# 86885974647565434342125458569795756674/torch.distributed.pipeline.sync.Pipe

Hardware: AMD Instinct MI355X
Metric: tokens/sec for 12-layer Transformer at PP=N (pipeline-parallel training) (higher is better)
Workload: dtype bf16

## Files before the change

mipipe/csrc/bindings.cpp:

```cpp
#include <torch/extension.h>
#include <ATen/hip/HIPContext.h>
#include <ATen/hip/HIPGeneratorImpl.h>
#include <ATen/core/Generator.h>
#include <ATen/hip/impl/HIPGuardImplMasqueradingAsCUDA.h>
#include <ATen/hip/impl/HIPStreamMasqueradingAsCUDA.h>

#include <mutex>
#include <optional>
#include <tuple>

#include "kernels/kernels.h"
#include "runtime/ipc.h"
#include "runtime/runtime.h"

namespace py = pybind11;
using at::Tensor;

namespace mipipe {
namespace {

#define MP_CHECK(cond, ...) TORCH_CHECK(cond, "mipipe: ", __VA_ARGS__)

hipStream_t cur_stream(const Tensor& t) { return at::hip::getCurrentHIPStreamMasqueradingAsCUDA(t.device().index()).stream(); }

// ... 1642 lines not shown
  MP_CHECK(t.scalar_type() == at::kFloat, who, ": sinks must be fp32, got ", t.scalar_type());
  MP_CHECK(t.dim() == 1 && t.size(0) == a.H, who, ": sinks must be [H] = [", a.H, "], one per query head");
  MP_CHECK(t.device() == q.device(), who, ": sinks must be on q's device");
  MP_CHECK(t.is_contiguous(), who, ": sinks must be contiguous");
  a.sinks = static_cast<const float*>(t.data_ptr());
}

void fill_options(AttnArgs& a, const char* who, const Tensor& q, bool causal, int64_t kv_len, int64_t window,
                  double softcap, const std::optional<Tensor>& doc_bounds, const std::optional<Tensor>& sinks) {
  attn_docs(a, who, doc_bounds, causal, q);
  attn_sinks(a, who, sinks, q);
  a.window = attn_window(who, window, causal, q, a.S);
  a.softcap = attn_softcap(who, softcap, q);
  MP_CHECK(kv_len == 0 || (q.scalar_type() == at::kFloat && kv_len > 0 && kv_len <= a.S), who,
           ": kv_len (a key-length bound) is for fp32, 0 < kv_len <= S");
  a.kv_len = (int)kv_len;
}

std::tuple<Tensor, Tensor, int64_t, int64_t, Tensor> py_attention_fwd(Tensor q, Tensor k, Tensor v, bool causal,
                                                                      double p, double scale, int64_t kv_len,
                                                                      std::optional<Tensor> words, int64_t words_seed,
                                                                      int64_t words_offset, int64_t window, double softcap,
                                                                      std::optional<Tensor> doc_bounds,
                                                                      std::optional<Tensor> sinks) {
  AttnArgs a;
  fill_qkv(a, q, k, v);
  fill_options(a, "attention", q, causal, kv_len, window, softcap, doc_bounds, sinks);
  MP_CHECK(p >= 0.0 && p < 1.0, "attention: bad dropout p");
  at::hip::HIPGuardMasqueradingAsCUDA guard(q.device());
  auto o = at::empty({a.B, a.S, a.H, a.D}, q.options());
  auto lse = at::empty({a.B, a.H, a.S}, q.options().dtype(at::kFloat));
  uint64_t seed = 0, offset = 0;
  if (p > 0.0) std::tie(seed, offset) = philox_draw(q.device(), 4);
  a.o = o.data_ptr(); a.sb_o = o.stride(0); a.ld_o = o.stride(1); a.sh_o = o.stride(2);
  a.lse = ptr<float>(lse);
  a.scale = (float)scale; a.p = (float)p; a.seed = seed; a.offset = offset; a.causal = causal;
  Tensor bits = at::empty({0}, q.options().dtype(at::kInt));
  if (q.scalar_type() == at::kFloat) {
    attention_f32_fwd(a, cur_stream(q));
  } else if (runs_long(a, q)) {
    bool reuse = false;
    if (p > 0.0) {
      const std::vector<int64_t> shape = {(int64_t)a.B * a.H, a.S / 32, a.S};
      reuse = words && words->defined() && words->sizes() == at::IntArrayRef(shape) &&
              words->scalar_type() == at::kInt && words->is_contiguous() && words->device() == q.device() &&
              (uint64_t)words_seed == seed && (uint64_t)words_offset == offset;
      bits = reuse ? *words : at::empty(shape, q.options().dtype(at::kInt));
      a.dmask = reinterpret_cast<uint32_t*>(bits.data_ptr());
    }
    if (reuse) attention_long_fwd_words(a, cur_stream(q));
    else attention_long_fwd(a, cur_stream(q));
  } else {
    attention_fwd(a, cur_stream(q));
// ... 288 lines not shown
  m.def("moe_combine_bwd", &py_moe_combine_bwd, py::arg("dy"), py::arg("ye"), py::arg("gate"), py::arg("src"));
  m.def("bias_act_fwd", &py_bias_act_fwd);
  m.def("softcap_fwd", &py_softcap_fwd, py::arg("x"), py::arg("cap"), py::arg("out") = py::none());
  m.def("softcap_bwd", &py_softcap_bwd, py::arg("dy"), py::arg("y"), py::arg("cap"), py::arg("out") = py::none());
  m.def("bias_act_bwd", &py_bias_act_bwd, py::arg("dy"), py::arg("saved"), py::arg("bias"), py::arg("act"),
        py::arg("p"), py::arg("seed"), py::arg("offset"), py::arg("need_dbias"), py::arg("dbias_acc") = py::none());
  m.def("column_sum", &py_column_sum, py::arg("x"), py::arg("out") = py::none(), py::arg("accumulate") = false);
  m.def("cross_entropy_fwd", &py_ce_fwd, py::arg("logits"), py::arg("target"), py::arg("ignore_index"),
        py::arg("t_offset") = 0);
  m.def("cross_entropy_bwd", &py_ce_bwd, py::arg("logits"), py::arg("target"), py::arg("lse"), py::arg("scale"),
        py::arg("ignore_index"), py::arg("row_scale") = py::none(), py::arg("out") = py::none(),
        py::arg("zero_pad") = false, py::arg("t_offset") = 0, py::arg("stat_out") = py::none());
  m.def("cross_entropy_mean_fwd", &py_ce_mean_fwd, py::arg("logits"), py::arg("target"), py::arg("ignore_index"));
  m.def("vsplit_head_fwd", &py_vsplit_head_fwd);
  m.def("vsplit_tail_fwd", &py_vsplit_tail_fwd);
  m.def("embedding_fwd", &py_embed_fwd);
  m.def("embedding_bwd", &py_embed_bwd, py::arg("tokens"), py::arg("dout"), py::arg("dweight"), py::arg("scale"),
        py::arg("p"), py::arg("seed"), py::arg("offset"), py::arg("dpe") = py::none());
  m.def("attention_supported", [](int64_t S, int64_t D) { return attention_supported((int)S, (int)D); });
  m.def("attention_f32_supported", [](int64_t S, int64_t D) { return attention_f32_supported((int)S, (int)D); });
  m.def("attention_fwd", &py_attention_fwd, py::arg("q"), py::arg("k"), py::arg("v"), py::arg("causal"), py::arg("p"),
        py::arg("scale"), py::arg("kv_len") = 0, py::arg("words") = py::none(), py::arg("words_seed") = 0,
        py::arg("words_offset") = 0, py::arg("window") = 0, py::arg("softcap") = 0.0,
        py::arg("doc_bounds") = py::none(), py::arg("sinks") = py::none());
  m.def("attention_bwd", &py_attention_bwd, py::arg("dout"), py::arg("q"), py::arg("k"), py::arg("v"), py::arg("o"),
        py::arg("lse"), py::arg("causal"), py::arg("p"), py::arg("scale"), py::arg("seed"), py::arg("offset"),
        py::arg("dq"), py::arg("dk"), py::arg("dv"), py::arg("bits") = py::none(), py::arg("kv_len") = 0,
        py::arg("window") = 0, py::arg("softcap") = 0.0, py::arg("doc_bounds") = py::none(),
        py::arg("sinks") = py::none(), py::arg("dsinks") = py::none(), py::arg("dsinks_accumulate") = false);
  m.def("attention_dsink", &py_attention_dsink, py::arg("lse"), py::arg("delta"), py::arg("sinks"), py::arg("dsinks"),
        py::arg("accumulate") = false);
  m.def("attention_long_supported", [](int64_t S, int64_t D) { return attention_long_supported((int)S, (int)D); });
  m.def("attention_long_set_fused_rng", &attention_long_set_fused_rng,
        "long-sequence attention: make the dropout keep words inside the forward kernel (true, default) or in a "
        "kernel of their own before it (false)");
  m.def("gemm_supported", &py_gemm_supported);
  m.def("gemm_f32_supported", &py_gemm_f32_supported);
  m.def("attention_set_fused_bwd", &attention_set_fused_bwd);
  m.def("gemm_set_rounds", &gemm_set_rounds,
        "multi-round GEMM grids whose last round is at most half full: 0 one launch, 1 (default) one launch per round "
        "of tiles when K >= 4096, 2 one launch per round at any K");
  m.def("gemm_set_splitk", &gemm_set_splitk, "split-K factor of under-filled long-K GEMMs: 0 off, 1 auto (default), n >= 2 forced");
  m.def("gemm_set_width", &gemm_set_width, "256-row GEMM block width: 0 auto (grid-quantisation rule), 128, 256");
  m.def("linear_fwd", &py_linear_fwd, py::arg("x"), py::arg("w"), py::arg("bias"), py::arg("act"), py::arg("p"),
        py::arg("save_preact"), py::arg("res") = py::none(), py::arg("xt") = py::none(),
        py::arg("aux_grad") = false, py::arg("bits") = py::none());
  m.def("linear_bits_ok",
        [](int64_t M, int64_t N, int64_t K, int64_t act, double p) {
          GemmArgs g;
          g.M = (int)M; g.N = (int)N; g.K = (int)K; g.act = (int)act; g.p = (float)p;
          g.a_kc = true; g.b_kc = true; g.epi = kEpiStoreAct;
          return gemm_supported(M, N, K) && gemm_bits_ok(g);
        },
        py::arg("M"), py::arg("N"), py::arg("K"), py::arg("act"), py::arg("p"),
        "whether linear_fwd can also write the ReLU output's nonzero mask as bits (kActReluBits)");
  m.def("gemm_emit_ok", &gemm_emit_ok, py::arg("act"), py::arg("p"), py::arg("aux"),
        "whether linear_fwd can also write x^T for this activation / dropout / pre-activation output");
  m.def("linear_wgrad_xt_segments", &py_linear_wgrad_xt_segments, py::arg("dys"), py::arg("xts"),
        py::arg("main_grad"), py::arg("accumulate") = true, py::arg("bias_grad") = py::none());
  m.def("linear_dgrad", &py_linear_dgrad, py::arg("dy"), py::arg("w"), py::arg("res") = py::none(),
        py::arg("out") = py::none(), py::arg("act") = 0, py::arg("saved") = py::none(), py::arg("p") = 0.0,
// ... 12 lines not shown
```

mipipe/csrc/kernels/attention.hip:

```cpp
#include <type_traits>

#include "common.h"
#include "kernels.h"

namespace mipipe {

namespace {

typedef __attribute__((ext_vector_type(4))) short s16x4;
typedef __attribute__((ext_vector_type(8))) short s16x8;
typedef __attribute__((address_space(3))) s16x4 lds_s16x4;

constexpr int kRows = 64;
constexpr int kThreads = 256;
constexpr float kLog2e = 1.4426950408889634f;

template <int D>
struct Img {
  static constexpr int kRowBytes = 2 * D;
  static constexpr int kChunks = D / 8;
  static constexpr int kBytes = kRows * kRowBytes;
  __device__ static __forceinline__ int f(int r) {
    if constexpr (kChunks >= 16) return (((r ^ (r >> 2)) & 1) << 1) | ((r & 2) << 1) | (r & 8);
    else if constexpr (kChunks == 8) return ((((r >> 1) ^ (r >> 2)) & 1) << 1) | ((r >> 1) & 4);
// ... 963 lines not shown
      dk[t2] = __builtin_amdgcn_mfma_f32_16x16x32_bf16(f1, frag_cols<D>(qimg, 16 * t2, 1, lane), dk[t2], 0, 0, 0);
    }
  }
  const DkvDst dst = dkv_dst<0>(blockIdx.y);
  bf16_t* dK = dst.dk;
  bf16_t* dV = dst.dv;
#pragma unroll
  for (int t2 = 0; t2 < ND; ++t2)
#pragma unroll
    for (int r = 0; r < 4; ++r) {
      const int64_t o = (int64_t)(key0 + r) * dst.ld + 16 * t2 + (lane & 15);
      dK[o] = f2bf(dk[t2][r] * a.scale);
      dV[o] = f2bf(dv[t2][r]);
    }
}

namespace shortseq {

constexpr int S = 128;
constexpr int kThreads = 512;
constexpr int kChunk = 64;
constexpr int kChunkImg = S * kChunk * 2;
constexpr int kSqImg = S * S * 2;
constexpr int kStageBytes = 3 * kChunkImg;
constexpr int kPOff = 4 * kChunkImg;
constexpr int kDsOff = kPOff + kSqImg;
constexpr int kSmem = kDsOff + kSqImg;
constexpr int kFwdPOff = 2 * kChunkImg;
constexpr int kFwdSmem = kFwdPOff + kSqImg;

__device__ __forceinline__ int coff(int r, int c16) { return Img<64>::off(r, c16); }
__device__ __forceinline__ int soff(int r, int c16) { return Img<128>::off(r, c16); }

__device__ __forceinline__ void load_chunk(const bf16_t* __restrict__ base, int64_t ld, int d0, int tid, uint4& v0,
                                           uint4& v1) {
  const int r = tid >> 3, c = tid & 7;
  v0 = *reinterpret_cast<const uint4*>(base + (int64_t)r * ld + d0 + 8 * c);
  v1 = *reinterpret_cast<const uint4*>(base + (int64_t)(r + 64) * ld + d0 + 8 * c);
}
__device__ __forceinline__ void store_chunk(char* img, int tid, const uint4& v0, const uint4& v1) {
  const int r = tid >> 3, c = tid & 7;
  *reinterpret_cast<uint4*>(img + coff(r, c)) = v0;
  *reinterpret_cast<uint4*>(img + coff(r + 64, c)) = v1;
}

__device__ __forceinline__ bf16x8 crow(const char* img, int rb, int s, int lane) {
  return *reinterpret_cast<const bf16x8*>(img + coff(rb + (lane & 15), 4 * s + (lane >> 4)));
}
__device__ __forceinline__ bf16x8 ccol(const char* img, int db, int s, int lane) {
  const int g = lane >> 4, q = (lane & 15) >> 2, p = lane & 3;
  const int r0 = 32 * s + 8 * g + q;
  const int c8 = (db >> 2) + p;
  const int o0 = coff(r0, c8 >> 1) + 8 * (c8 & 1);
  const int o1 = coff(r0 + 4, c8 >> 1) + 8 * (c8 & 1);
  const s16x4 lo = __builtin_amdgcn_ds_read_tr16_b64_v4i16((lds_s16x4*)(img + o0));
  const s16x4 hi = __builtin_amdgcn_ds_read_tr16_b64_v4i16((lds_s16x4*)(img + o1));
  return __builtin_bit_cast(bf16x8, __builtin_shufflevector(lo, hi, 0, 1, 2, 3, 4, 5, 6, 7));
}
__device__ __forceinline__ bf16x8 srow(const char* img, int rb, int s, int lane) {
  return *reinterpret_cast<const bf16x8*>(img + soff(rb + (lane & 15), 4 * s + (lane >> 4)));
}
__device__ __forceinline__ bf16x8 scol(const char* img, int ib, int s, int lane) {
  const int g = lane >> 4, q = (lane & 15) >> 2, p = lane & 3;
  const int r0 = 32 * s + 8 * g + q;
  const int c8 = (ib >> 2) + p;
  const int o0 = soff(r0, c8 >> 1) + 8 * (c8 & 1);
  const int o1 = soff(r0 + 4, c8 >> 1) + 8 * (c8 & 1);
  const s16x4 lo = __builtin_amdgcn_ds_read_tr16_b64_v4i16((lds_s16x4*)(img + o0));
  const s16x4 hi = __builtin_amdgcn_ds_read_tr16_b64_v4i16((lds_s16x4*)(img + o1));
  return __builtin_bit_cast(bf16x8, __builtin_shufflevector(lo, hi, 0, 1, 2, 3, 4, 5, 6, 7));
}

template <int D, bool CAUSAL>
__global__ void __launch_bounds__(kThreads, 1) attn_bwd_s128_kernel(AttnArgs a) {
  extern __shared__ __attribute__((aligned(16))) char smem[];
  const int tid = threadIdx.x, lane = tid & 63, wave = __builtin_amdgcn_readfirstlane(tid >> 6);
  const int bh = blockIdx.x;
  const int b = bh / a.H, h = bh % a.H;
  const int64_t boff = (int64_t)b * a.sb_qkv + (int64_t)h * a.sh_qkv;
  const int64_t koff = (int64_t)b * a.sb_qkv + (int64_t)kv_head(a, h) * a.sh_qkv;
  const bf16_t* Q = reinterpret_cast<const bf16_t*>(a.q) + boff;
  const bf16_t* K = reinterpret_cast<const bf16_t*>(a.k) + koff;
  const bf16_t* V = reinterpret_cast<const bf16_t*>(a.v) + koff;
  const bf16_t* dO = reinterpret_cast<const bf16_t*>(a.dout) + (int64_t)b * a.sb_o + (int64_t)h * a.sh_o;
  constexpr int NC = D / kChunk;

  f32x4 sacc[8], pacc[8];
#pragma unroll
  for (int j = 0; j < 8; ++j) sacc[j] = pacc[j] = f32x4{0.f, 0.f, 0.f, 0.f};
  const int myrow = wave * 16 + (lane & 15);
  const bf16_t* qrow = Q + (int64_t)myrow * a.ld_qkv;
  const bf16_t* drow = dO + (int64_t)myrow * a.ld_o;

  uint4 k0, k1, v0, v1;
  load_chunk(K, a.ld_qkv, 0, tid, k0, k1);
  load_chunk(V, a.ld_qkv, 0, tid, v0, v1);
  store_chunk(smem, tid, k0, k1);
  store_chunk(smem + kChunkImg, tid, v0, v1);
  __syncthreads();
#pragma unroll 1
  for (int c = 0; c < NC; ++c) {
    const char* kimg = smem + (c & 1) * 2 * kChunkImg;
    const char* vimg = kimg + kChunkImg;
    if (c + 1 < NC) {
      load_chunk(K, a.ld_qkv, (c + 1) * kChunk, tid, k0, k1);
      load_chunk(V, a.ld_qkv, (c + 1) * kChunk, tid, v0, v1);
    }
    bf16x8 qf[2], df[2];
#pragma unroll
    for (int s2 = 0; s2 < 2; ++s2) {
      qf[s2] = frag_global(qrow + c * kChunk, s2, lane);
      df[s2] = frag_global(drow + c * kChunk, s2, lane);
    }
#pragma unroll
    for (int s2 = 0; s2 < 2; ++s2)
#pragma unroll
      for (int j = 0; j < 8; ++j) {
        sacc[j] = __builtin_amdgcn_mfma_f32_16x16x32_bf16(qf[s2], crow(kimg, 16 * j, s2, lane), sacc[j], 0, 0, 0);
        pacc[j] = __builtin_amdgcn_mfma_f32_16x16x32_bf16(df[s2], crow(vimg, 16 * j, s2, lane), pacc[j], 0, 0, 0);
      }
    if (c + 1 < NC) {
      char* nimg = smem + ((c + 1) & 1) * 2 * kChunkImg;
      store_chunk(nimg, tid, k0, k1);
      store_chunk(nimg + kChunkImg, tid, v0, v1);
    }
    __syncthreads();
  }

  const int qrow0 = wave * 16 + 4 * (lane >> 4);
  const float sl2 = a.scale * kLog2e;
  const float pscale = a.p > 0.f ? 1.f / (1.f - a.p) : 1.f;
  float lse2[4];
#pragma unroll
  for (int r = 0; r < 4; ++r) lse2[r] = a.lse[(int64_t)bh * S + qrow0 + r] * kLog2e;
  float dsum[4] = {0.f, 0.f, 0.f, 0.f};
#pragma unroll
  for (int j = 0; j < 8; ++j) {
    const int key = 16 * j + (lane & 15);
    uint32_t w[4] = {0xFFFFFFFFu, 0xFFFFFFFFu, 0xFFFFFFFFu, 0xFFFFFFFFu};
    if (a.p > 0.f) {
      const uint4 mw = attn_mask_words(a, bh, qrow0 >> 2, key);
      w[0] = mw.x; w[1] = mw.y; w[2] = mw.z; w[3] = mw.w;
    }
#pragma unroll
    for (int r = 0; r < 4; ++r) {
      float pr = __builtin_amdgcn_exp2f(sacc[j][r] * sl2 - lse2[r]);
      if (CAUSAL && key > qrow0 + r) pr = 0.f;
      float dp = pacc[j][r];
      float pd = pr;
      if (a.p > 0.f) {
        const bool keep = w[r] >= a.threshold;
        dp = keep ? dp * pscale : 0.f;
        pd = keep ? pr * pscale : 0.f;
      }
      sacc[j][r] = pr;
      pacc[j][r] = dp;
      dsum[r] += pr * dp;
      *reinterpret_cast<bf16_t*>(smem + kPOff + soff(qrow0 + r, key >> 3) + 2 * (key & 7)) = f2bf(pd);
    }
  }
  float delta[4];
#pragma unroll
  for (int r = 0; r < 4; ++r) delta[r] = row_reduce_sum16(dsum[r]);
#pragma unroll
  for (int j = 0; j < 8; ++j) {
    const int key = 16 * j + (lane & 15);
#pragma unroll
    for (int r = 0; r < 4; ++r) {
      const float ds = sacc[j][r] * (pacc[j][r] - delta[r]);
      *reinterpret_cast<bf16_t*>(smem + kDsOff + soff(qrow0 + r, key >> 3) + 2 * (key & 7)) = f2bf(ds);
    }
  }

  const char* pimg = smem + kPOff;
  const char* dsimg = smem + kDsOff;
  char* kimg = smem;
  char* qimg = smem + kChunkImg;
  char* dimg = smem + 2 * kChunkImg;
  const int r0 = wave * 16;
  uint4 a0, a1, b0, b1, e0, e1;
  load_chunk(K, a.ld_qkv, 0, tid, a0, a1);
  load_chunk(Q, a.ld_qkv, 0, tid, b0, b1);
  load_chunk(dO, a.ld_o, 0, tid, e0, e1);
#pragma unroll 1
  for (int c = 0; c < NC; ++c) {
    const int d0 = c * kChunk;
    __syncthreads();
    store_chunk(kimg, tid, a0, a1);
    store_chunk(qimg, tid, b0, b1);
    store_chunk(dimg, tid, e0, e1);
    __syncthreads();
    if (c + 1 < NC) {
      load_chunk(K, a.ld_qkv, d0 + kChunk, tid, a0, a1);
      load_chunk(Q, a.ld_qkv, d0 + kChunk, tid, b0, b1);
      load_chunk(dO, a.ld_o, d0 + kChunk, tid, e0, e1);
    }
    f32x4 dq[4], dk[4], dv[4];
#pragma unroll
    for (int t = 0; t < 4; ++t) dq[t] = dk[t] = dv[t] = f32x4{0.f, 0.f, 0.f, 0.f};
#pragma unroll
    for (int ks = 0; ks < 4; ++ks) {
      const bf16x8 a_dq = srow(dsimg, r0, ks, lane);
      const bf16x8 a_dk = scol(dsimg, r0, ks, lane);
      const bf16x8 a_dv = scol(pimg, r0, ks, lane);
#pragma unroll
      for (int t = 0; t < 4; ++t) {
        dq[t] = __builtin_amdgcn_mfma_f32_16x16x32_bf16(a_dq, ccol(kimg, 16 * t, ks, lane), dq[t], 0, 0, 0);
        dk[t] = __builtin_amdgcn_mfma_f32_16x16x32_bf16(a_dk, ccol(qimg, 16 * t, ks, lane), dk[t], 0, 0, 0);
        dv[t] = __builtin_amdgcn_mfma_f32_16x16x32_bf16(a_dv, ccol(dimg, 16 * t, ks, lane), dv[t], 0, 0, 0);
      }
    }
    const int orow = r0 + 4 * (lane >> 4);
    __syncthreads();
#pragma unroll
    for (int t = 0; t < 4; ++t) {
      const int col = 16 * t + (lane & 15);
#pragma unroll
      for (int r = 0; r < 4; ++r) {
        const int at = coff(orow + r, col >> 3) + 2 * (col & 7);
        *reinterpret_cast<bf16_t*>(kimg + at) = f2bf(dq[t][r] * a.scale);
        *reinterpret_cast<bf16_t*>(qimg + at) = f2bf(dk[t][r] * a.scale);
        *reinterpret_cast<bf16_t*>(dimg + at) = f2bf(dv[t][r]);
      }
    }
    __syncthreads();
    {
      const int r = tid >> 3, cc = tid & 7;
      const DkvDst dst = dkv_dst<0>(blockIdx.x);
      bf16_t* dK = dst.dk;
      bf16_t* dV = dst.dv;
      bf16_t* dQ = dq_dst<0>(blockIdx.x);
#pragma unroll
      for (int h2 = 0; h2 < 2; ++h2) {
        const int row = r + 64 * h2;
        const int off = coff(row, cc);
        const int64_t g = (int64_t)row * a.ld_qkv + d0 + 8 * cc;
        const int64_t gk = (int64_t)row * dst.ld + d0 + 8 * cc;
        *reinterpret_cast<uint4*>(dQ + g) = *reinterpret_cast<const uint4*>(kimg + off);
        *reinterpret_cast<uint4*>(dK + gk) = *reinterpret_cast<const uint4*>(qimg + off);
        *reinterpret_cast<uint4*>(dV + gk) = *reinterpret_cast<const uint4*>(dimg + off);
      }
    }
  }
}

template <int D, bool CAUSAL>
__global__ void __launch_bounds__(kThreads, 2) attn_fwd_s128_kernel(AttnArgs a) {
  extern __shared__ __attribute__((aligned(16))) char smem[];
  const int tid = threadIdx.x, lane = tid & 63, wave = __builtin_amdgcn_readfirstlane(tid >> 6);
  const int bh = blockIdx.x;
  const int b = bh / a.H, h = bh % a.H;
  const int64_t boff = (int64_t)b * a.sb_qkv + (int64_t)h * a.sh_qkv;
  const int64_t koff = (int64_t)b * a.sb_qkv + (int64_t)kv_head(a, h) * a.sh_qkv;
  const bf16_t* Q = reinterpret_cast<const bf16_t*>(a.q) + boff;
  const bf16_t* K = reinterpret_cast<const bf16_t*>(a.k) + koff;
  const bf16_t* V = reinterpret_cast<const bf16_t*>(a.v) + koff;
  constexpr int NC = D / kChunk;

  f32x4 sacc[8];
#pragma unroll
  for (int j = 0; j < 8; ++j) sacc[j] = f32x4{0.f, 0.f, 0.f, 0.f};
  const bf16_t* qrow = Q + (int64_t)(wave * 16 + (lane & 15)) * a.ld_qkv;

  uint4 k0, k1;
  load_chunk(K, a.ld_qkv, 0, tid, k0, k1);
// ... 92 lines not shown
#pragma unroll
    for (int t = 0; t < 4; ++t)
#pragma unroll
      for (int r = 0; r < 4; ++r)
        O[(int64_t)(orow + r) * a.ld_o + c * kChunk + 16 * t + (lane & 15)] = f2bf(o[t][r]);
    if (c + 1 < NC) store_chunk(smem + ((c + 1) & 1) * kChunkImg, tid, v0, v1);
    __syncthreads();
  }
}

}

template <int D>
size_t fwd_smem() { return 2 * Img<D>::kBytes + 4 * 16 * kScrStride * 2; }
template <int D>
size_t dkdv_smem() { return fwd_smem<D>() + 128 * sizeof(float); }

int g_attn_fused_bwd = 1;
const int g_attn_wide = [] {
  const char* e = getenv("MIPIPE_ATTN_WIDE");
  return e == nullptr ? 1 : atoi(e);
}();

template <typename Kern>
void set_smem(Kern k, size_t bytes) {
  hipFuncSetAttribute(reinterpret_cast<const void*>(k), hipFuncAttributeMaxDynamicSharedMemorySize, (int)bytes);
}

template <int D, bool CAUSAL>
void run_fwd(const AttnArgs& a, hipStream_t s) {
  if (a.S == shortseq::S && g_attn_fused_bwd) {
    static bool once_s = false;
    if (!once_s) {
      set_smem(shortseq::attn_fwd_s128_kernel<D, CAUSAL>, shortseq::kFwdSmem);
      once_s = true;
    }
    hipLaunchKernelGGL((shortseq::attn_fwd_s128_kernel<D, CAUSAL>), dim3(a.B * a.H), dim3(shortseq::kThreads),
                       shortseq::kFwdSmem, s, a);
    return;
  }
  if (D == 64 && a.S % kWideRows == 0 && g_attn_wide) {
    static bool once_w = false;
    if (!once_w) { set_smem(attn_fwd_wide_kernel<CAUSAL>, wide_fwd_smem()); once_w = true; }
    hipLaunchKernelGGL((attn_fwd_wide_kernel<CAUSAL>), dim3(a.S / kWideRows, a.B * a.H), dim3(kThreads),
                       wide_fwd_smem(), s, a);
    return;
  }
  const size_t sm = fwd_smem<D>();
  static bool once = false;
  if (!once) { set_smem(attn_fwd_kernel<D, CAUSAL>, sm); once = true; }
  hipLaunchKernelGGL((attn_fwd_kernel<D, CAUSAL>), dim3(a.S / kRows, a.B * a.H), dim3(kThreads), sm, s, a);
}

template <int D, bool CAUSAL>
void run_bwd(const AttnArgs& a, hipStream_t s) {
  const size_t sm = fwd_smem<D>(), sm2 = dkdv_smem<D>();
  static bool once = false;
  if (!once) {
    set_smem(attn_dq_kernel<D, CAUSAL>, sm);
    set_smem(attn_dkdv_kernel<D, CAUSAL>, sm2);
    once = true;
  }
  if (a.S == shortseq::S && g_attn_fused_bwd) {
    static bool once_s = false;
    if (!once_s) {
      set_smem(shortseq::attn_bwd_s128_kernel<D, CAUSAL>, shortseq::kSmem);
      once_s = true;
    }
    hipLaunchKernelGGL((shortseq::attn_bwd_s128_kernel<D, CAUSAL>), dim3(a.B * a.H), dim3(shortseq::kThreads),
                       shortseq::kSmem, s, a);
    return;
  }
  const int64_t rows = (int64_t)a.B * a.S * a.H;
  hipLaunchKernelGGL(attn_delta_kernel, dim3((unsigned)((rows + 3) / 4)), dim3(256), 0, s, a, D);
  hipLaunchKernelGGL((attn_dkdv_kernel<D, CAUSAL>), dim3(a.S / kRows, a.B * a.H), dim3(kThreads), sm2, s, a);
  if (D == 64 && a.S % kWideRows == 0 && g_attn_wide) {
    static bool once_w = false;
    if (!once_w) { set_smem(attn_dq_wide_kernel<CAUSAL>, wide_fwd_smem()); once_w = true; }
    hipLaunchKernelGGL((attn_dq_wide_kernel<CAUSAL>), dim3(a.S / kWideRows, a.B * a.H), dim3(kThreads),
                       wide_fwd_smem(), s, a);
    return;
  }
  hipLaunchKernelGGL((attn_dq_kernel<D, CAUSAL>), dim3(a.S / kRows, a.B * a.H), dim3(kThreads), sm, s, a);
}

template <int D, bool CAUSAL, bool WINDOW, bool SOFTCAP, bool DOCS, bool SINK>
void launch_fwd_generic(const AttnArgs& a, hipStream_t s) {
  const size_t sm = fwd_smem<D>();
  static bool once = false;
  if (!once) { set_smem(attn_fwd_kernel<D, CAUSAL, WINDOW, SOFTCAP, DOCS, SINK>, sm); once = true; }
  hipLaunchKernelGGL((attn_fwd_kernel<D, CAUSAL, WINDOW, SOFTCAP, DOCS, SINK>), dim3(a.S / kRows, a.B * a.H),
                     dim3(kThreads), sm, s, a);
}
// ... 44 lines not shown
  else if (D == 128) f(std::integral_constant<int, 128>{});
  else f(std::integral_constant<int, 256>{});
}

template <typename F>
void with_flag(bool on, F&& f) {
  if (on) f(std::true_type{});
  else f(std::false_type{});
}

template <typename F>
void with_mask(const AttnArgs& a, F&& f) {
  using Y = std::true_type;
  using N = std::false_type;
  if (a.doc_start != nullptr) f(Y{}, N{}, Y{});
  else if (a.window > 0) f(Y{}, Y{}, N{});
  else if (a.causal) f(Y{}, N{}, N{});
  else f(N{}, N{}, N{});
}

}

void attention_set_fused_bwd(int on) { g_attn_fused_bwd = on; }

void attention_dsink(const float* lse, const float* delta, const float* sinks, float* dsinks, int B, int H, int S,
                     bool accumulate, hipStream_t s) {
  hipLaunchKernelGGL(attn_dsink_kernel, dim3(H), dim3(kThreads), 0, s, lse, delta, sinks, dsinks, B, H, S,
                     accumulate ? 1 : 0);
}

bool attention_supported(int S, int D) { return S > 0 && S % kRows == 0 && (D == 64 || D == 128 || D == 256); }

void attention_fwd(const AttnArgs& ai, hipStream_t s) {
  const AttnArgs a = prepared(ai);
  with_d(a.D, [&](auto d) {
    constexpr int D = decltype(d)::value;
    if (!is_generic(a)) {
      with_flag(a.causal, [&](auto causal) { run_fwd<D, decltype(causal)::value>(a, s); });
      return;
    }
    with_mask(a, [&](auto causal, auto window, auto docs) {
      with_flag(a.softcap > 0.f, [&](auto cap) {
        with_flag(a.sinks != nullptr, [&](auto sink) {
          launch_fwd_generic<D, decltype(causal)::value, decltype(window)::value, decltype(cap)::value,
                             decltype(docs)::value, decltype(sink)::value>(a, s);
        });
// ... 24 lines not shown
```

mipipe/csrc/kernels/kernels.h:

```cpp
#pragma once

#include <hip/hip_runtime.h>
#include <stdint.h>

namespace mipipe {

typedef uint16_t bf16_t;

template <typename T>
struct LnArgs {
  const T* x = nullptr;
  const T* res = nullptr;
  const T* gamma = nullptr;
  const T* beta = nullptr;
  T* y = nullptr;
  T* z = nullptr;
  float* mean = nullptr;
  float* rstd = nullptr;
  int rows = 0, cols = 0;
  float eps = 1e-5f;
  float p = 0.f;
  uint64_t seed = 0, offset = 0;
};

// ... 260 lines not shown
  const auto* ap = attn_args_late<kArgOffset>();
  const int H = ap->H, b = bh / H, h = bh - b * H;
  const int64_t off = (int64_t)b * ap->sb_dkv + (int64_t)h * ap->sh_dkv;
  return DkvDst{reinterpret_cast<bf16_t*>(ap->dk) + off, reinterpret_cast<bf16_t*>(ap->dv) + off, ap->ld_dkv};
}
template <int kArgOffset>
__device__ __forceinline__ bf16_t* dq_dst(int bh) {
  const auto* ap = attn_args_late<kArgOffset>();
  const int H = ap->H, b = bh / H, h = bh - b * H;
  return reinterpret_cast<bf16_t*>(ap->dq) + (int64_t)b * ap->sb_qkv + (int64_t)h * ap->sh_qkv;
}
#endif
inline AttnArgs attn_resolved(const AttnArgs& ai) {
  AttnArgs a = ai;
  if (a.group < 1) a.group = 1;
  a.group_rcp = ((1u << 20) + (uint32_t)a.group - 1) / (uint32_t)a.group;
  if (a.ld_dkv == 0 && a.sb_dkv == 0 && a.sh_dkv == 0) {
    a.ld_dkv = a.ld_qkv; a.sb_dkv = a.sb_qkv; a.sh_dkv = a.sh_qkv;
  }
  return a;
}
bool attention_supported(int S, int D);
void attention_set_fused_bwd(int on);
void attention_fwd(const AttnArgs& a, hipStream_t s);
void attention_bwd(const AttnArgs& a, hipStream_t s);
void attention_dsink(const float* lse, const float* delta, const float* sinks, float* dsinks, int B, int H, int S,
                     bool accumulate, hipStream_t s);
bool attention_f32_supported(int S, int D);
bool attention_long_supported(int S, int D);
void attention_long_set_fused_rng(bool on);
void attention_long_fwd(const AttnArgs& a, hipStream_t s);
void attention_long_fwd_words(const AttnArgs& a, hipStream_t s);
void attention_long_bwd(const AttnArgs& a, hipStream_t s);
void attention_f32_fwd(const AttnArgs& a, hipStream_t s);
void attention_f32_bwd(const AttnArgs& a, hipStream_t s);

template <typename T>
void cross_entropy_fwd(const T* logits, const int64_t* target, int64_t rows, int64_t V, int64_t ld,
                       int64_t ignore_index, float* loss, float* lse, hipStream_t s, int64_t t_offset = 0);
template <typename T>
void cross_entropy_mean_fwd(const T* logits, const int64_t* target, int64_t rows, int64_t V, int64_t ld,
                            int64_t ignore_index, float* loss_row, float* lse, float* weight, float* loss,
                            hipStream_t s);
template <typename T>
void cross_entropy_bwd(const T* logits, const int64_t* target, const float* lse, const float* scale,
                       const float* row_scale, int64_t rows, int64_t V, int64_t ld, int64_t ld_out,
// ... 37 lines not shown
```

Before: 161,900.

## Make S=128 attention backward persistent with register-ring prefetch of next head

The fused short-sequence attention backward now launches at most one block per CU and loops over (batch, head) pairs. It keeps all K and V chunks resident in LDS and prefetches the next item's chunks and Q/dO fragments through a two-slot register ring, so global loads overlap the MFMA work. This is meant to cut per-block launch and load latency and improve overlap, at the cost of more registers, the whole 160 KiB of LDS at D=256, and a grid-size knob. The change also adds an optional preallocated output tensor to attention_fwd.

```diff
diff --git a/mipipe/csrc/bindings.cpp b/mipipe/csrc/bindings.cpp
--- a/mipipe/csrc/bindings.cpp
+++ b/mipipe/csrc/bindings.cpp
@@ -1688,13 +1688,21 @@
                                                                       std::optional<Tensor> words, int64_t words_seed,
                                                                       int64_t words_offset, int64_t window, double softcap,
                                                                       std::optional<Tensor> doc_bounds,
-                                                                      std::optional<Tensor> sinks) {
+                                                                      std::optional<Tensor> sinks,
+                                                                      std::optional<Tensor> out) {
   AttnArgs a;
   fill_qkv(a, q, k, v);
   fill_options(a, "attention", q, causal, kv_len, window, softcap, doc_bounds, sinks);
   MP_CHECK(p >= 0.0 && p < 1.0, "attention: bad dropout p");
   at::hip::HIPGuardMasqueradingAsCUDA guard(q.device());
-  auto o = at::empty({a.B, a.S, a.H, a.D}, q.options());
+  const bool have_out = out && out->defined();
+  if (have_out) {
+    check_bshd(*out, "out");
+    MP_CHECK(out->sizes() == at::IntArrayRef({(int64_t)a.B, (int64_t)a.S, (int64_t)a.H, (int64_t)a.D}) &&
+                 out->scalar_type() == q.scalar_type() && out->device() == q.device(),
+             "attention: out must be [B, S, H, D] of q's dtype on q's device");
+  }
+  auto o = have_out ? *out : at::empty({a.B, a.S, a.H, a.D}, q.options());
   auto lse = at::empty({a.B, a.H, a.S}, q.options().dtype(at::kFloat));
   uint64_t seed = 0, offset = 0;
   if (p > 0.0) std::tie(seed, offset) = philox_draw(q.device(), 4);
@@ -2029,7 +2037,7 @@
   m.def("attention_fwd", &py_attention_fwd, py::arg("q"), py::arg("k"), py::arg("v"), py::arg("causal"), py::arg("p"),
         py::arg("scale"), py::arg("kv_len") = 0, py::arg("words") = py::none(), py::arg("words_seed") = 0,
         py::arg("words_offset") = 0, py::arg("window") = 0, py::arg("softcap") = 0.0,
-        py::arg("doc_bounds") = py::none(), py::arg("sinks") = py::none());
+        py::arg("doc_bounds") = py::none(), py::arg("sinks") = py::none(), py::arg("out") = py::none());
   m.def("attention_bwd", &py_attention_bwd, py::arg("dout"), py::arg("q"), py::arg("k"), py::arg("v"), py::arg("o"),
         py::arg("lse"), py::arg("causal"), py::arg("p"), py::arg("scale"), py::arg("seed"), py::arg("offset"),
         py::arg("dq"), py::arg("dk"), py::arg("dv"), py::arg("bits") = py::none(), py::arg("kv_len") = 0,
@@ -2044,6 +2052,7 @@
   m.def("gemm_supported", &py_gemm_supported);
   m.def("gemm_f32_supported", &py_gemm_f32_supported);
   m.def("attention_set_fused_bwd", &attention_set_fused_bwd);
+  m.def("attention_set_s128_grid", &attention_set_s128_grid, py::arg("n"));
   m.def("gemm_set_rounds", &gemm_set_rounds,
         "multi-round GEMM grids whose last round is at most half full: 0 one launch, 1 (default) one launch per round "
         "of tiles when K >= 4096, 2 one launch per round at any K");
diff --git a/mipipe/csrc/kernels/attention.hip b/mipipe/csrc/kernels/attention.hip
--- a/mipipe/csrc/kernels/attention.hip
+++ b/mipipe/csrc/kernels/attention.hip
@@ -1009,10 +1009,11 @@
 constexpr int kChunk = 64;
 constexpr int kChunkImg = S * kChunk * 2;
 constexpr int kSqImg = S * S * 2;
-constexpr int kStageBytes = 3 * kChunkImg;
-constexpr int kPOff = 4 * kChunkImg;
-constexpr int kDsOff = kPOff + kSqImg;
-constexpr int kSmem = kDsOff + kSqImg;
+template <int D> constexpr int kPOff = (D / kChunk) * kChunkImg;
+template <int D> constexpr int kDsOff = kPOff<D> + kSqImg;
+template <int D> constexpr int kSpOff = kDsOff<D> + kSqImg;
+template <int D> constexpr int kSmem = kSpOff<D> + 2 * kChunkImg;
+static_assert(kSmem<256> == 160 * 1024, "the D = 256 backward fills a CU's LDS exactly");
 constexpr int kFwdPOff = 2 * kChunkImg;
 constexpr int kFwdSmem = kFwdPOff + kSqImg;
 
@@ -1058,176 +1059,244 @@
   return __builtin_bit_cast(bf16x8, __builtin_shufflevector(lo, hi, 0, 1, 2, 3, 4, 5, 6, 7));
 }
 
+typedef __attribute__((ext_vector_type(4))) uint32_t u32x4;
+struct ChunkPair {
+  u32x4 a0, a1, b0, b1;
+};
+__device__ __forceinline__ void load_pair(const bf16_t* __restrict__ A, int64_t lda, const bf16_t* __restrict__ B,
+                                          int64_t ldb, int d0, int tid, ChunkPair& p) {
+  const int r = tid >> 3, c = tid & 7;
+  p.a0 = *reinterpret_cast<const u32x4*>(A + (int64_t)r * lda + d0 + 8 * c);
+  p.a1 = *reinterpret_cast<const u32x4*>(A + (int64_t)(r + 64) * lda + d0 + 8 * c);
+  p.b0 = *reinterpret_cast<const u32x4*>(B + (int64_t)r * ldb + d0 + 8 * c);
+  p.b1 = *reinterpret_cast<const u32x4*>(B + (int64_t)(r + 64) * ldb + d0 + 8 * c);
+}
+__device__ __forceinline__ void store_pair(char* aimg, char* bimg, int tid, const ChunkPair& p) {
+  const int r = tid >> 3, c = tid & 7;
+  *reinterpret_cast<u32x4*>(aimg + coff(r, c)) = p.a0;
+  *reinterpret_cast<u32x4*>(aimg + coff(r + 64, c)) = p.a1;
+  *reinterpret_cast<u32x4*>(bimg + coff(r, c)) = p.b0;
+  *reinterpret_cast<u32x4*>(bimg + coff(r + 64, c)) = p.b1;
+}
+
+__device__ __forceinline__ int opaque(int v) {
+  asm volatile("" : "+v"(v));
+  return v;
+}
+
+struct BwdHead {
+  const bf16_t* Q;
+  const bf16_t* K;
+  const bf16_t* V;
+  const bf16_t* dO;
+};
+__device__ __forceinline__ BwdHead bwd_head(const AttnArgs& a, int bh) {
+  const int b = bh / a.H, h = bh % a.H;
+  const int64_t boff = (int64_t)b * a.sb_qkv + (int64_t)h * a.sh_qkv;
+  const int64_t koff = (int64_t)b * a.sb_qkv + (int64_t)kv_head(a, h) * a.sh_qkv;
+  return BwdHead{reinterpret_cast<const bf16_t*>(a.q) + boff, reinterpret_cast<const bf16_t*>(a.k) + koff,
+                 reinterpret_cast<const bf16_t*>(a.v) + koff,
+                 reinterpret_cast<const bf16_t*>(a.dout) + (int64_t)b * a.sb_o + (int64_t)h * a.sh_o};
+}
+template <int NC>
+__device__ __forceinline__ void load_item(const AttnArgs& a, const BwdHead& hd, int i, int tid, ChunkPair& p) {
+  if (i < NC) load_pair(hd.K, a.ld_qkv, hd.V, a.ld_qkv, i * kChunk, tid, p);
+  else load_pair(hd.Q, a.ld_qkv, hd.dO, a.ld_o, (i - NC) * kChunk, tid, p);
+}
+template <int NC>
+__device__ __forceinline__ void refill(const AttnArgs& a, const BwdHead& hd, int bh, int i, int tid, ChunkPair& p) {
+  if (i + 2 < 2 * NC) {
+    load_item<NC>(a, hd, i + 2, tid, p);
+  } else if (bh + (int)gridDim.x < a.B * a.H) {
+    load_item<NC>(a, bwd_head(a, bh + (int)gridDim.x), i + 2 - 2 * NC, tid, p);
+  }
+}
+template <int NC>
+__device__ __forceinline__ void store_refill(const AttnArgs& a, const BwdHead& hd, int bh, int i, int tid, char* aimg,
+                                             char* bimg, ChunkPair& ring0, ChunkPair& ring1) {
+  if ((i & 1) == 0) {
+    store_pair(aimg, bimg, tid, ring0);
+    refill<NC>(a, hd, bh, i, tid, ring0);
+  } else {
+    store_pair(aimg, bimg, tid, ring1);
+    refill<NC>(a, hd, bh, i, tid, ring1);
+  }
+}
+
+template <int NC>
+__device__ __forceinline__ void load_afrags(const AttnArgs& a, const BwdHead& hd, int row, int lane,
+                                            bf16x8 (&qf)[NC][2], bf16x8 (&df)[NC][2]) {
+  const bf16_t* qrow = hd.Q + (int64_t)row * a.ld_qkv;
+  const bf16_t* drow = hd.dO + (int64_t)row * a.ld_o;
+#pragma unroll
+  for (int c = 0; c < NC; ++c)
+#pragma unroll
+    for (int s2 = 0; s2 < 2; ++s2) {
+      qf[c][s2] = frag_global(qrow + c * kChunk, s2, lane);
+      df[c][s2] = frag_global(drow + c * kChunk, s2, lane);
+    }
+}
+
 template <int D, bool CAUSAL>
 __global__ void __launch_bounds__(kThreads, 1) attn_bwd_s128_kernel(AttnArgs a) {
   extern __shared__ __attribute__((aligned(16))) char smem[];
-  const int tid = threadIdx.x, lane = tid & 63, wave = __builtin_amdgcn_readfirstlane(tid >> 6);
-  const int bh = blockIdx.x;
-  const int b = bh / a.H, h = bh % a.H;
-  const int64_t boff = (int64_t)b * a.sb_qkv + (int64_t)h * a.sh_qkv;
-  const int64_t koff = (int64_t)b * a.sb_qkv + (int64_t)kv_head(a, h) * a.sh_qkv;
-  const bf16_t* Q = reinterpret_cast<const bf16_t*>(a.q) + boff;
-  const bf16_t* K = reinterpret_cast<const bf16_t*>(a.k) + koff;
-  const bf16_t* V = reinterpret_cast<const bf16_t*>(a.v) + koff;
-  const bf16_t* dO = reinterpret_cast<const bf16_t*>(a.dout) + (int64_t)b * a.sb_o + (int64_t)h * a.sh_o;
+  int tid = threadIdx.x;
   constexpr int NC = D / kChunk;
-
-  f32x4 sacc[8], pacc[8];
-#pragma unroll
-  for (int j = 0; j < 8; ++j) sacc[j] = pacc[j] = f32x4{0.f, 0.f, 0.f, 0.f};
-  const int myrow = wave * 16 + (lane & 15);
-  const bf16_t* qrow = Q + (int64_t)myrow * a.ld_qkv;
-  const bf16_t* drow = dO + (int64_t)myrow * a.ld_o;
-
-  uint4 k0, k1, v0, v1;
-  load_chunk(K, a.ld_qkv, 0, tid, k0, k1);
-  load_chunk(V, a.ld_qkv, 0, tid, v0, v1);
-  store_chunk(smem, tid, k0, k1);
-  store_chunk(smem + kChunkImg, tid, v0, v1);
-  __syncthreads();
+  const int nbh = a.B * a.H, step = gridDim.x;
+  char* const spq = smem + kSpOff<D>;
+  char* const spd = spq + kChunkImg;
+  const char* const pimg = smem + kPOff<D>;
+  const char* const dsimg = smem + kDsOff<D>;
+
+  ChunkPair ring0, ring1;
+  bf16x8 qf[NC][2], df[NC][2];
+  int bh = blockIdx.x;
+  {
+    const BwdHead hd = bwd_head(a, bh);
+    load_item<NC>(a, hd, 0, tid, ring0);
+    load_item<NC>(a, hd, 1, tid, ring1);
+    load_afrags<NC>(a, hd, (tid >> 6) * 16 + (tid & 15), tid & 63, qf, df);
+  }
 #pragma unroll 1
-  for (int c = 0; c < NC; ++c) {
-    const char* kimg = smem + (c & 1) * 2 * kChunkImg;
-    const char* vimg = kimg + kChunkImg;
-    if (c + 1 < NC) {
-      load_chunk(K, a.ld_qkv, (c + 1) * kChunk, tid, k0, k1);
-      load_chunk(V, a.ld_qkv, (c + 1) * kChunk, tid, v0, v1);
-    }
-    bf16x8 qf[2], df[2];
-#pragma unroll
-    for (int s2 = 0; s2 < 2; ++s2) {
-      qf[s2] = frag_global(qrow + c * kChunk, s2, lane);
-      df[s2] = frag_global(drow + c * kChunk, s2, lane);
-    }
-#pragma unroll
-    for (int s2 = 0; s2 < 2; ++s2)
-#pragma unroll
-      for (int j = 0; j < 8; ++j) {
-        sacc[j] = __builtin_amdgcn_mfma_f32_16x16x32_bf16(qf[s2], crow(kimg, 16 * j, s2, lane), sacc[j], 0, 0, 0);
-        pacc[j] = __builtin_amdgcn_mfma_f32_16x16x32_bf16(df[s2], crow(vimg, 16 * j, s2, lane), pacc[j], 0, 0, 0);
-      }
-    if (c + 1 < NC) {
-      char* nimg = smem + ((c + 1) & 1) * 2 * kChunkImg;
-      store_chunk(nimg, tid, k0, k1);
-      store_chunk(nimg + kChunkImg, tid, v0, v1);
-    }
+  for (; bh < nbh; bh += step) {
+    tid = opaque(tid);
+    const int lane = tid & 63, wave = __builtin_amdgcn_readfirstlane(tid >> 6);
+    const BwdHead hd = bwd_head(a, bh);
+    const int qrow0 = wave * 16 + 4 * (lane >> 4);
+
+    float lse2[4];
+#pragma unroll
+    for (int r = 0; r < 4; ++r) lse2[r] = a.lse[(int64_t)bh * S + qrow0 + r];
+    f32x4 sacc[8], pacc[8];
+#pragma unroll
+    for (int j = 0; j < 8; ++j) sacc[j] = pacc[j] = f32x4{0.f, 0.f, 0.f, 0.f};
+
+    store_refill<NC>(a, hd, bh, 0, tid, smem, smem + kPOff<D>, ring0, ring1);
     __syncthreads();
-  }
-
-  const int qrow0 = wave * 16 + 4 * (lane >> 4);
-  const float sl2 = a.scale * kLog2e;
-  const float pscale = a.p > 0.f ? 1.f / (1.f - a.p) : 1.f;
-  float lse2[4];
-#pragma unroll
-  for (int r = 0; r < 4; ++r) lse2[r] = a.lse[(int64_t)bh * S + qrow0 + r] * kLog2e;
-  float dsum[4] = {0.f, 0.f, 0.f, 0.f};
-#pragma unroll
-  for (int j = 0; j < 8; ++j) {
-    const int key = 16 * j + (lane & 15);
-    uint32_t w[4] = {0xFFFFFFFFu, 0xFFFFFFFFu, 0xFFFFFFFFu, 0xFFFFFFFFu};
-    if (a.p > 0.f) {
-      const uint4 mw = attn_mask_words(a, bh, qrow0 >> 2, key);
-      w[0] = mw.x; w[1] = mw.y; w[2] = mw.z; w[3] = mw.w;
-    }
-#pragma unroll
-    for (int r = 0; r < 4; ++r) {
-      float pr = __builtin_amdgcn_exp2f(sacc[j][r] * sl2 - lse2[r]);
-      if (CAUSAL && key > qrow0 + r) pr = 0.f;
-      float dp = pacc[j][r];
-      float pd = pr;
+#pragma unroll
+    for (int c = 0; c < NC; ++c) {
+      const char* kimg = smem + c * kChunkImg;
+      const char* vimg = smem + kPOff<D> + c * kChunkImg;
+      const int tid_c = opaque(tid), lane_c = tid_c & 63;
+#pragma unroll
+      for (int s2 = 0; s2 < 2; ++s2)
+#pragma unroll
+        for (int j = 0; j < 8; ++j) {
+          sacc[j] = __builtin_amdgcn_mfma_f32_16x16x32_bf16(qf[c][s2], crow(kimg, 16 * j, s2, lane_c), sacc[j], 0, 0, 0);
+          pacc[j] = __builtin_amdgcn_mfma_f32_16x16x32_bf16(df[c][s2], crow(vimg, 16 * j, s2, lane_c), pacc[j], 0, 0, 0);
+        }
+      if (c + 1 < NC) {
+        store_refill<NC>(a, hd, bh, c + 1, tid_c, smem + (c + 1) * kChunkImg, smem + kPOff<D> + (c + 1) * kChunkImg,
+                         ring0, ring1);
+      } else {
+        store_refill<NC>(a, hd, bh, NC, tid_c, spq, spd, ring0, ring1);
+      }
+      __syncthreads();
+    }
+
+    const float sl2 = a.scale * kLog2e;
+    const float pscale = a.p > 0.f ? 1.f / (1.f - a.p) : 1.f;
+#pragma unroll
+    for (int r = 0; r < 4; ++r) lse2[r] *= kLog2e;
+    float dsum[4] = {0.f, 0.f, 0.f, 0.f};
+#pragma unroll
+    for (int j = 0; j < 8; ++j) {
+      const int key = 16 * j + (lane & 15);
+      uint32_t w[4] = {0xFFFFFFFFu, 0xFFFFFFFFu, 0xFFFFFFFFu, 0xFFFFFFFFu};
       if (a.p > 0.f) {
-        const bool keep = w[r] >= a.threshold;
-        dp = keep ? dp * pscale : 0.f;
-        pd = keep ? pr * pscale : 0.f;
-      }
-      sacc[j][r] = pr;
-      pacc[j][r] = dp;
-      dsum[r] += pr * dp;
-      *reinterpret_cast<bf16_t*>(smem + kPOff + soff(qrow0 + r, key >> 3) + 2 * (key & 7)) = f2bf(pd);
-    }
-  }
-  float delta[4];
-#pragma unroll
-  for (int r = 0; r < 4; ++r) delta[r] = row_reduce_sum16(dsum[r]);
-#pragma unroll
-  for (int j = 0; j < 8; ++j) {
-    const int key = 16 * j + (lane & 15);
-#pragma unroll
-    for (int r = 0; r < 4; ++r) {
-      const float ds = sacc[j][r] * (pacc[j][r] - delta[r]);
-      *reinterpret_cast<bf16_t*>(smem + kDsOff + soff(qrow0 + r, key >> 3) + 2 * (key & 7)) = f2bf(ds);
-    }
-  }
-
-  const char* pimg = smem + kPOff;
-  const char* dsimg = smem + kDsOff;
-  char* kimg = smem;
-  char* qimg = smem + kChunkImg;
-  char* dimg = smem + 2 * kChunkImg;
-  const int r0 = wave * 16;
-  uint4 a0, a1, b0, b1, e0, e1;
-  load_chunk(K, a.ld_qkv, 0, tid, a0, a1);
-  load_chunk(Q, a.ld_qkv, 0, tid, b0, b1);
-  load_chunk(dO, a.ld_o, 0, tid, e0, e1);
-#pragma unroll 1
-  for (int c = 0; c < NC; ++c) {
-    const int d0 = c * kChunk;
+        const uint4 mw = attn_mask_words(a, bh, qrow0 >> 2, key);
+        w[0] = mw.x; w[1] = mw.y; w[2] = mw.z; w[3] = mw.w;
+      }
+#pragma unroll
+      for (int r = 0; r < 4; ++r) {
+        float pr = __builtin_amdgcn_exp2f(sacc[j][r] * sl2 - lse2[r]);
+        if (CAUSAL && key > qrow0 + r) pr = 0.f;
+        float dp = pacc[j][r];
+        float pd = pr;
+        if (a.p > 0.f) {
+          const bool keep = w[r] >= a.threshold;
+          dp = keep ? dp * pscale : 0.f;
+          pd = keep ? pr * pscale : 0.f;
+        }
+        sacc[j][r] = pr;
+        pacc[j][r] = dp;
+        dsum[r] += pr * dp;
+        *reinterpret_cast<bf16_t*>(smem + kPOff<D> + soff(qrow0 + r, key >> 3) + 2 * (key & 7)) = f2bf(pd);
+      }
+    }
+    float delta[4];
+#pragma unroll
+    for (int r = 0; r < 4; ++r) delta[r] = row_reduce_sum16(dsum[r]);
+#pragma unroll
+    for (int j = 0; j < 8; ++j) {
+      const int key = 16 * j + (lane & 15);
+#pragma unroll
+      for (int r = 0; r < 4; ++r) {
+        const float ds = sacc[j][r] * (pacc[j][r] - delta[r]);
+        *reinterpret_cast<bf16_t*>(smem + kDsOff<D> + soff(qrow0 + r, key >> 3) + 2 * (key & 7)) = f2bf(ds);
+      }
+    }
+
+    const int r0 = wave * 16;
+    if (bh + step < nbh) load_afrags<NC>(a, bwd_head(a, bh + step), wave * 16 + (lane & 15), lane, qf, df);
+#pragma unroll
+    for (int c = 0; c < NC; ++c) {
+      const int d0 = c * kChunk;
+      char* kimg = smem + c * kChunkImg;
+      const int tid_c = opaque(tid), lane_c = tid_c & 63;
+      if (c > 0) {
+        __syncthreads();
+        store_refill<NC>(a, hd, bh, NC + c, tid_c, spq, spd, ring0, ring1);
+      }
+      __syncthreads();
+      f32x4 dq[4], dk[4], dv[4];
+#pragma unroll
+      for (int t = 0; t < 4; ++t) dq[t] = dk[t] = dv[t] = f32x4{0.f, 0.f, 0.f, 0.f};
+#pragma unroll
+      for (int ks = 0; ks < 4; ++ks) {
+        const bf16x8 a_dq = srow(dsimg, r0, ks, lane_c);
+        const bf16x8 a_dk = scol(dsimg, r0, ks, lane_c);
+        const bf16x8 a_dv = scol(pimg, r0, ks, lane_c);
+#pragma unroll
+        for (int t = 0; t < 4; ++t) {
+          dq[t] = __builtin_amdgcn_mfma_f32_16x16x32_bf16(a_dq, ccol(kimg, 16 * t, ks, lane_c), dq[t], 0, 0, 0);
+          dk[t] = __builtin_amdgcn_mfma_f32_16x16x32_bf16(a_dk, ccol(spq, 16 * t, ks, lane_c), dk[t], 0, 0, 0);
+          dv[t] = __builtin_amdgcn_mfma_f32_16x16x32_bf16(a_dv, ccol(spd, 16 * t, ks, lane_c), dv[t], 0, 0, 0);
+        }
+      }
+      const int orow = r0 + 4 * (lane_c >> 4);
+      __syncthreads();
+#pragma unroll
+      for (int t = 0; t < 4; ++t) {
+        const int col = 16 * t + (lane_c & 15);
+#pragma unroll
+        for (int r = 0; r < 4; ++r) {
+          const int at = coff(orow + r, col >> 3) + 2 * (col & 7);
+          *reinterpret_cast<bf16_t*>(kimg + at) = f2bf(dq[t][r] * a.scale);
+          *reinterpret_cast<bf16_t*>(spq + at) = f2bf(dk[t][r] * a.scale);
+          *reinterpret_cast<bf16_t*>(spd + at) = f2bf(dv[t][r]);
+        }
+      }
+      __syncthreads();
+      {
+        const int r = tid_c >> 3, cc8 = tid_c & 7;
+        const DkvDst dst = dkv_dst<0>(bh);
+        bf16_t* dK = dst.dk;
+        bf16_t* dV = dst.dv;
+        bf16_t* dQ = dq_dst<0>(bh);
+#pragma unroll
+        for (int h2 = 0; h2 < 2; ++h2) {
+          const int row = r + 64 * h2;
+          const int off = coff(row, cc8);
+          const int64_t g = (int64_t)row * a.ld_qkv + d0 + 8 * cc8;
+          const int64_t gk = (int64_t)row * dst.ld + d0 + 8 * cc8;
+          *reinterpret_cast<uint4*>(dQ + g) = *reinterpret_cast<const uint4*>(kimg + off);
+          *reinterpret_cast<uint4*>(dK + gk) = *reinterpret_cast<const uint4*>(spq + off);
+          *reinterpret_cast<uint4*>(dV + gk) = *reinterpret_cast<const uint4*>(spd + off);
+        }
+      }
+    }
     __syncthreads();
-    store_chunk(kimg, tid, a0, a1);
-    store_chunk(qimg, tid, b0, b1);
-    store_chunk(dimg, tid, e0, e1);
-    __syncthreads();
-    if (c + 1 < NC) {
-      load_chunk(K, a.ld_qkv, d0 + kChunk, tid, a0, a1);
-      load_chunk(Q, a.ld_qkv, d0 + kChunk, tid, b0, b1);
-      load_chunk(dO, a.ld_o, d0 + kChunk, tid, e0, e1);
-    }
-    f32x4 dq[4], dk[4], dv[4];
-#pragma unroll
-    for (int t = 0; t < 4; ++t) dq[t] = dk[t] = dv[t] = f32x4{0.f, 0.f, 0.f, 0.f};
-#pragma unroll
-    for (int ks = 0; ks < 4; ++ks) {
-      const bf16x8 a_dq = srow(dsimg, r0, ks, lane);
-      const bf16x8 a_dk = scol(dsimg, r0, ks, lane);
-      const bf16x8 a_dv = scol(pimg, r0, ks, lane);
-#pragma unroll
-      for (int t = 0; t < 4; ++t) {
-        dq[t] = __builtin_amdgcn_mfma_f32_16x16x32_bf16(a_dq, ccol(kimg, 16 * t, ks, lane), dq[t], 0, 0, 0);
-        dk[t] = __builtin_amdgcn_mfma_f32_16x16x32_bf16(a_dk, ccol(qimg, 16 * t, ks, lane), dk[t], 0, 0, 0);
-        dv[t] = __builtin_amdgcn_mfma_f32_16x16x32_bf16(a_dv, ccol(dimg, 16 * t, ks, lane), dv[t], 0, 0, 0);
-      }
-    }
-    const int orow = r0 + 4 * (lane >> 4);
-    __syncthreads();
-#pragma unroll
-    for (int t = 0; t < 4; ++t) {
-      const int col = 16 * t + (lane & 15);
-#pragma unroll
-      for (int r = 0; r < 4; ++r) {
-        const int at = coff(orow + r, col >> 3) + 2 * (col & 7);
-        *reinterpret_cast<bf16_t*>(kimg + at) = f2bf(dq[t][r] * a.scale);
-        *reinterpret_cast<bf16_t*>(qimg + at) = f2bf(dk[t][r] * a.scale);
-        *reinterpret_cast<bf16_t*>(dimg + at) = f2bf(dv[t][r]);
-      }
-    }
-    __syncthreads();
-    {
-      const int r = tid >> 3, cc = tid & 7;
-      const DkvDst dst = dkv_dst<0>(blockIdx.x);
-      bf16_t* dK = dst.dk;
-      bf16_t* dV = dst.dv;
-      bf16_t* dQ = dq_dst<0>(blockIdx.x);
-#pragma unroll
-      for (int h2 = 0; h2 < 2; ++h2) {
-        const int row = r + 64 * h2;
-        const int off = coff(row, cc);
-        const int64_t g = (int64_t)row * a.ld_qkv + d0 + 8 * cc;
-        const int64_t gk = (int64_t)row * dst.ld + d0 + 8 * cc;
-        *reinterpret_cast<uint4*>(dQ + g) = *reinterpret_cast<const uint4*>(kimg + off);
-        *reinterpret_cast<uint4*>(dK + gk) = *reinterpret_cast<const uint4*>(qimg + off);
-        *reinterpret_cast<uint4*>(dV + gk) = *reinterpret_cast<const uint4*>(dimg + off);
-      }
-    }
   }
 }
 
@@ -1366,6 +1435,19 @@
   return e == nullptr ? 1 : atoi(e);
 }();
 
+int g_attn_s128_grid = 0;
+int s128_grid(int heads) {
+  static const int cus = [] {
+    int dev = 0, n = 0;
+    if (hipGetDevice(&dev) != hipSuccess ||
+        hipDeviceGetAttribute(&n, hipDeviceAttributeMultiprocessorCount, dev) != hipSuccess || n <= 0)
+      n = 256;
+    return n;
+  }();
+  const int want = g_attn_s128_grid > 0 ? g_attn_s128_grid : cus;
+  return want < heads ? want : heads;
+}
+
 template <typename Kern>
 void set_smem(Kern k, size_t bytes) {
   hipFuncSetAttribute(reinterpret_cast<const void*>(k), hipFuncAttributeMaxDynamicSharedMemorySize, (int)bytes);
@@ -1408,11 +1490,11 @@
   if (a.S == shortseq::S && g_attn_fused_bwd) {
     static bool once_s = false;
     if (!once_s) {
-      set_smem(shortseq::attn_bwd_s128_kernel<D, CAUSAL>, shortseq::kSmem);
+      set_smem(shortseq::attn_bwd_s128_kernel<D, CAUSAL>, shortseq::kSmem<D>);
       once_s = true;
     }
-    hipLaunchKernelGGL((shortseq::attn_bwd_s128_kernel<D, CAUSAL>), dim3(a.B * a.H), dim3(shortseq::kThreads),
-                       shortseq::kSmem, s, a);
+    hipLaunchKernelGGL((shortseq::attn_bwd_s128_kernel<D, CAUSAL>), dim3(s128_grid(a.B * a.H)),
+                       dim3(shortseq::kThreads), shortseq::kSmem<D>, s, a);
     return;
   }
   const int64_t rows = (int64_t)a.B * a.S * a.H;
@@ -1503,6 +1585,7 @@
 }
 
 void attention_set_fused_bwd(int on) { g_attn_fused_bwd = on; }
+void attention_set_s128_grid(int n) { g_attn_s128_grid = n > 0 ? n : 0; }
 
 void attention_dsink(const float* lse, const float* delta, const float* sinks, float* dsinks, int B, int H, int S,
                      bool accumulate, hipStream_t s) {
diff --git a/mipipe/csrc/kernels/kernels.h b/mipipe/csrc/kernels/kernels.h
--- a/mipipe/csrc/kernels/kernels.h
+++ b/mipipe/csrc/kernels/kernels.h
@@ -306,6 +306,7 @@
 }
 bool attention_supported(int S, int D);
 void attention_set_fused_bwd(int on);
+void attention_set_s128_grid(int n);
 void attention_fwd(const AttnArgs& a, hipStream_t s);
 void attention_bwd(const AttnArgs& a, hipStream_t s);
 void attention_dsink(const float* lse, const float* delta, const float* sinks, float* dsinks, int B, int H, int S,
```

Measured after the change: 162,400 (median of 6 runs). No clear change (+0.3%).
